# penn-graphics-research/HOT

Hardware: AMD Instinct MI355X
Metric: ms per nonlinear (L-BFGS) iteration; P2G+G2P Mparticles/s; achieved HBM GB/s vs roofline (lower is better)
Workload: dtype f64; 1 GPU; C2: one 63^3-cell cube x 8 ppc (63^3 cells per GPU), fixed-corotated E=50000 nu=0.3, dx=0.01, dt=1/24, -lsolver 3 -mg_level 3 -smoother 5 -coarseSolver 2 --project --linesearch --bcproject --usecn -cneps 1e-7; particles_per_gpu=2000376, particles_total=2000376, nodes_total=267565, levels=3, parallelism=1 GPU

## Files before the change

hot_amd/csrc/mg_build.hip:

```cpp
#include "hot_impl.h"
#include "hot_svd.h"
#include <rocprim/rocprim.hpp>

namespace hot {

__global__ void k_hash_clear2(HashMap h)
{
    uint32_t i = blockIdx.x * blockDim.x + threadIdx.x;
    if (i > h.mask) return;
    h.keys[i] = ~0ULL;
    h.minrank[i] = ~0ULL;
    h.id[i] = -1;
}
__global__ void k_coord_map_insert(HashMap h, const int32_t* __restrict__ coord, int n)
{
    int i = blockIdx.x * blockDim.x + threadIdx.x;
    if (i >= n) return;
    uint32_t s = hash_insert_min(h, coord_key(coord[3 * i], coord[3 * i + 1], coord[3 * i + 2]), (unsigned long long)i);
    h.id[s] = i;
}

__device__ __forceinline__ bool parent_of(const int32_t* __restrict__ coord, int s, int& px, int& py, int& pz)
{
    int i = s >> 3, l = s & 7;
    int x = coord[3 * i], y = coord[3 * i + 1], z = coord[3 * i + 2];
    int dx = l >> 2, dy = (l >> 1) & 1, dz = l & 1;
    if ((dx && !(x & 1)) || (dy && !(y & 1)) || (dz && !(z & 1))) return false;
    px = x / 2 + dx, py = y / 2 + dy, pz = z / 2 + dz;
    return true;
}
__global__ void k_coarse_insert(HashMap h, const int32_t* __restrict__ coord, int n)
{
    int s = blockIdx.x * blockDim.x + threadIdx.x;
    if (s >= n * 8) return;
    int px, py, pz;
    if (parent_of(coord, s, px, py, pz)) hash_insert_min(h, coord_key(px, py, pz), (unsigned long long)s);
}
__global__ void k_coarse_flag(HashMap h, const int32_t* __restrict__ coord, int32_t* flags, int n)
{
    int s = blockIdx.x * blockDim.x + threadIdx.x;
    if (s >= n * 8) return;
    int px, py, pz;
    int f = 0;
    if (parent_of(coord, s, px, py, pz)) {
        int32_t slot = hash_find_slot(h, coord_key(px, py, pz));
        f = h.minrank[slot] == (unsigned long long)s;
    }
    flags[s] = f;
}
__global__ void k_coarse_assign(HashMap h, const int32_t* __restrict__ coord, const int32_t* __restrict__ flags, const int32_t* __restrict__ scan, int32_t* ccoord, int n)
{
    int s = blockIdx.x * blockDim.x + threadIdx.x;
    if (s >= n * 8 || !flags[s]) return;
    int px, py, pz;
    parent_of(coord, s, px, py, pz);
    int id = scan[s];
    h.id[hash_find_slot(h, coord_key(px, py, pz))] = id;
    ccoord[3 * id] = px, ccoord[3 * id + 1] = py, ccoord[3 * id + 2] = pz;
}
template <class T>
__global__ void k_build_P(HashMap cmap, const int32_t* __restrict__ coord, int32_t* pcol, T* pw, int n)
{
    int i = blockIdx.x * blockDim.x + threadIdx.x;
    if (i >= n) return;
    int x = coord[3 * i], y = coord[3 * i + 1], z = coord[3 * i + 2];
    int first = hash_find_id(cmap, coord_key(x / 2, y / 2, z / 2));
    for (int l = 0; l < 8; ++l) {
        int dx = l >> 2, dy = (l >> 1) & 1, dz = l & 1;
        T wx = (x & 1) ? (T)0.5 : (dx ? (T)0 : (T)1), wy = (y & 1) ? (T)0.5 : (dy ? (T)0 : (T)1), wz = (z & 1) ? (T)0.5 : (dz ? (T)0 : (T)1);
        T w = wx * wy * wz;
        int c = first;
        if (w != (T)0) c = hash_find_id(cmap, coord_key(x / 2 + dx, y / 2 + dy, z / 2 + dz));
        pcol[8 * (int64_t)i + l] = c;
        pw[8 * (int64_t)i + l] = w;
    }
}
__global__ void k_build_children(HashMap fmap, const int32_t* __restrict__ ccoord, int32_t* child, int nc)
{
    int e = blockIdx.x * blockDim.x + threadIdx.x;
    if (e >= nc * 27) return;
    int I = e / 27, q = e - I * 27;
    int a = q / 9 - 1, b = (q / 3) % 3 - 1, c = q % 3 - 1;
    int x = 2 * ccoord[3 * I] + a, y = 2 * ccoord[3 * I + 1] + b, z = 2 * ccoord[3 * I + 2] + c;
    child[e] = (x | y | z) < 0 ? -1 : hash_find_id(fmap, coord_key(x, y, z));
}
__global__ void k_coarse_cols(HashMap cmap, const int32_t* __restrict__ ccoord, int32_t* col, int nc)
{
    int64_t e = (int64_t)blockIdx.x * blockDim.x + threadIdx.x;
    if (e >= (int64_t)nc * 125) return;
    int n = (int)(e / 125), k = (int)(e - (int64_t)n * 125);
    int x = ccoord[3 * n] - (k / 25 - 2), y = ccoord[3 * n + 1] - ((k / 5) % 5 - 2), z = ccoord[3 * n + 2] - (k % 5 - 2);
    int j = (x | y | z) < 0 ? -1 : hash_find_id(cmap, coord_key(x, y, z));
    col[e] = j >= 0 ? j : (n > 0 ? 0 : 1);
}

__device__ __forceinline__ void ap_window(int x, int y, int z, int& na, int& nb, int& nc) { na = 3 + (x & 1), nb = 3 + (y & 1), nc = 3 + (z & 1); }
template <class T>
__global__ __launch_bounds__(256) void k_ap(const int32_t* __restrict__ coord, const T* __restrict__ val, T* ap, int n, const uint8_t* __restrict__ own)
{
    __shared__ T row[4][1125];
    int w = threadIdx.x >> 6, lane = threadIdx.x & 63;
    int i = blockIdx.x * 4 + w;
    if (own && i < n && !own[i]) i = n;
    if (i < n) {
        const T* src = val + (int64_t)i * 1125;
        for (int e = lane; e < 1125; e += 64) row[w][e] = src[e];
    }
    __syncthreads();
    if (i >= n) return;
    int x = coord[3 * i], y = coord[3 * i + 1], z = coord[3 * i + 2];
    int cbx = (x - 2) >> 1, cby = (y - 2) >> 1, cbz = (z - 2) >> 1;
    int na, nb, nc;
    ap_window(x, y, z, na, nb, nc);
    const int cnt9 = na * nb * nc * 9;
    for (int o = lane; o < cnt9; o += 64) {
        int js = o / 9, comp = o - js * 9;
        int a = js / (nb * nc), b = (js / nc) % nb, c = js % nc;
        int Jx = cbx + a, Jy = cby + b, Jz = cbz + c;
        T sum = (T)0;
#pragma unroll
        for (int da = -1; da <= 1; ++da) {
            int ddx = x - (2 * Jx + da);
            if (ddx < -2 || ddx > 2) continue;
#pragma unroll
            for (int db = -1; db <= 1; ++db) {
                int ddy = y - (2 * Jy + db);
                if (ddy < -2 || ddy > 2) continue;
#pragma unroll
                for (int dc = -1; dc <= 1; ++dc) {
                    int ddz = z - (2 * Jz + dc);
                    if (ddz < -2 || ddz > 2) continue;
                    T wgt = (da ? (T)0.5 : (T)1) * (db ? (T)0.5 : (T)1) * (dc ? (T)0.5 : (T)1);
                    sum += wgt * row[w][((ddx + 2) * 25 + (ddy + 2) * 5 + (ddz + 2)) * 9 + comp];
                }
            }
        }
        ap[(int64_t)i * 576 + o] = sum;
    }
}
__global__ void k_ap_cols(HashMap cmap, const int32_t* __restrict__ coord, int32_t* apc, int n)
{
    int64_t e = (int64_t)blockIdx.x * blockDim.x + threadIdx.x;
    if (e >= (int64_t)n * 64) return;
    int i = (int)(e >> 6), js = (int)(e & 63);
    int na, nb, nc;
    ap_window(coord[3 * i], coord[3 * i + 1], coord[3 * i + 2], na, nb, nc);
    if ((js >> 4) >= na || ((js >> 2) & 3) >= nb || (js & 3) >= nc) {
        apc[e] = -1;
        return;
    }
    int Jx = ((coord[3 * i] - 2) >> 1) + (js >> 4), Jy = ((coord[3 * i + 1] - 2) >> 1) + ((js >> 2) & 3), Jz = ((coord[3 * i + 2] - 2) >> 1) + (js & 3);
    int j = (Jx | Jy | Jz) < 0 ? -1 : hash_find_id(cmap, coord_key(Jx, Jy, Jz));
    apc[e] = j >= 0 ? j : 0;
}
template <class T>
__global__ __launch_bounds__(256) void k_rap(const int32_t* __restrict__ ccoord, const int32_t* __restrict__ child, const T* __restrict__ ap, T* cval, int nc,
    const uint8_t* __restrict__ fine_own )
{
    __shared__ T sap[9 * 576];
    __shared__ int32_t sci[27];
    const int tid = threadIdx.x, I = blockIdx.x;
    if (tid < 27) {
        const int ci = child[I * 27 + tid];
        sci[tid] = (ci < 0 || (fine_own && !fine_own[ci])) ? -1 : ci;
    }
    int kx[5], ky[5], kz[5], comp[5];
    T sum[5];
#pragma unroll
    for (int t = 0; t < 5; ++t) {
        const int o = min(tid + 256 * t, 1124), k = o / 9;
        comp[t] = o - 9 * k, kx[t] = k / 25, ky[t] = (k / 5) % 5, kz[t] = k % 5, sum[t] = (T)0;
    }
    __syncthreads();
#pragma unroll
    for (int batch = 0; batch < 3; ++batch) {
        for (int e = tid; e < 9 * 576; e += 256) {
            const int q = 9 * batch + e / 576, ci = sci[q];
            const int cnt9 = (3 + (q / 9 != 1)) * (3 + ((q / 3) % 3 != 1)) * (3 + (q % 3 != 1)) * 9;
            if (e % 576 < cnt9) sap[e] = ci >= 0 ? ap[(int64_t)ci * 576 + e % 576] : (T)0;
        }
        __syncthreads();
#pragma unroll
        for (int qq = 0; qq < 9; ++qq) {
            const int q = 9 * batch + qq, da = q / 9 - 1, db = (q / 3) % 3 - 1, dc = q % 3 - 1;
            if (sci[q] < 0) continue;
            const T wgt = (da ? (T)0.5 : (T)1) * (db ? (T)0.5 : (T)1) * (dc ? (T)0.5 : (T)1);
            const int na = 3 + (da != 0), nb = 3 + (db != 0), nc = 3 + (dc != 0);
#pragma unroll
            for (int t = 0; t < 5; ++t) {
                const int a = 3 - kx[t] + (da < 0), bb = 3 - ky[t] + (db < 0), c = 3 - kz[t] + (dc < 0);
                if ((unsigned)a >= (unsigned)na || (unsigned)bb >= (unsigned)nb || (unsigned)c >= (unsigned)nc) continue;
                sum[t] += wgt * sap[qq * 576 + ((a * nb + bb) * nc + c) * 9 + comp[t]];
            }
        }
        __syncthreads();
    }
#pragma unroll
    for (int t = 0; t < 5; ++t)
        if (tid + 256 * t < 1125) cval[(int64_t)I * 1125 + tid + 256 * t] = sum[t];
}

__global__ void k_color_insert(HashMap h, const int32_t* __restrict__ coord, int n)
{
    int i = blockIdx.x * blockDim.x + threadIdx.x;
    if (i >= n) return;
    hash_insert_min(h, coord_key(coord[3 * i] >> 2, coord[3 * i + 1] >> 2, coord[3 * i + 2] >> 2), (unsigned long long)i);
}
__device__ __forceinline__ int color_of(const int32_t* __restrict__ coord, int i)
{
    return (((coord[3 * i] >> 2) & 1) << 2) | (((coord[3 * i + 1] >> 2) & 1) << 1) | ((coord[3 * i + 2] >> 2) & 1);
}
__global__ void k_color_flag(HashMap h, const int32_t* __restrict__ coord, int32_t* flags, int n)
{
    int e = blockIdx.x * blockDim.x + threadIdx.x;
    if (e >= 8 * n) return;
    int c = e / n, i = e - c * n;
    int f = 0;
    if (color_of(coord, i) == c) {
        int32_t slot = hash_find_slot(h, coord_key(coord[3 * i] >> 2, coord[3 * i + 1] >> 2, coord[3 * i + 2] >> 2));
        f = h.minrank[slot] == (unsigned long long)i;
    }
    flags[e] = f;
}
__global__ void k_color_assign(HashMap h, const int32_t* __restrict__ coord, const int32_t* __restrict__ flags, const int32_t* __restrict__ scan, int n)
{
    int e = blockIdx.x * blockDim.x + threadIdx.x;
    if (e >= 8 * n || !flags[e]) return;
    int c = e / n, i = e - c * n;
    int32_t slot = hash_find_slot(h, coord_key(coord[3 * i] >> 2, coord[3 * i + 1] >> 2, coord[3 * i + 2] >> 2));
    h.id[slot] = scan[e] - scan[c * n];
}
__global__ void k_color_keys(HashMap h, const int32_t* __restrict__ coord, uint64_t* keys, uint32_t* vals, int n)
{
    int i = blockIdx.x * blockDim.x + threadIdx.x;
    if (i >= n) return;
    int32_t bid = hash_find_id(h, coord_key(coord[3 * i] >> 2, coord[3 * i + 1] >> 2, coord[3 * i + 2] >> 2));
    keys[i] = ((uint64_t)color_of(coord, i) << 56) | ((uint64_t)(uint32_t)bid << 32) | (uint32_t)i;
    vals[i] = (uint32_t)i;
}
__global__ void k_color_heads(const uint64_t* __restrict__ keys, int32_t* flags, int n)
{
    int p = blockIdx.x * blockDim.x + threadIdx.x;
    if (p >= n) return;
    flags[p] = (p == 0 || (keys[p] >> 32) != (keys[p - 1] >> 32)) ? 1 : 0;
}
__global__ void k_color_finish(const uint64_t* __restrict__ keys, const int32_t* __restrict__ flags, const int32_t* __restrict__ scan, int32_t* gs_order, int32_t* block_start,
    int32_t* color_begin, int n, int nblocks)
{
    int p = blockIdx.x * blockDim.x + threadIdx.x;
    if (p >= n) return;
    gs_order[p] = (int32_t)(keys[p] & 0xffffffffu);
    if (p == 0) block_start[nblocks] = n;
    if (flags[p]) {
        int b = scan[p];
        block_start[b] = p;
        int c = (int)(keys[p] >> 56);
        int cprev = p == 0 ? -1 : (int)(keys[p - 1] >> 56);
        for (int cc = cprev + 1; cc <= c; ++cc) color_begin[cc] = b;
    }
    if (p == n - 1) {
        int c = (int)(keys[p] >> 56);
        for (int cc = c + 1; cc <= 8; ++cc) color_begin[cc] = nblocks;
    }
}
__global__ void k_color_ckey(const uint64_t* __restrict__ keys, const int32_t* __restrict__ scan, const int32_t* __restrict__ block_start, uint32_t* ckey, int n)
{
    int p = blockIdx.x * blockDim.x + threadIdx.x;
    if (p >= n) return;
    int node = (int)(keys[p] & 0xffffffffu);
    int lo = 0, hi = 0;
    (void)lo, (void)hi;
    uint32_t color = (uint32_t)(keys[p] >> 56), bid = (uint32_t)((keys[p] >> 32) & 0xffffff);
    int b = scan[p];
    int start = block_start[b] == p ? p : block_start[b - 1];
    ckey[node] = (color << 28) | (bid << 7) | (uint32_t)(p - start + 1);
}

template <class T>
static void build_coord_map(Ctx<T>* ctx, Level<T>& L)
{
    uint32_t cap = 1024;
    while (cap < 2u * (uint32_t)L.n + 16u) cap <<= 1;
    L.hkeys.reserve(cap), L.hrank.reserve(cap), L.hid.reserve(cap);
    L.map.keys = L.hkeys.p, L.map.minrank = L.hrank.p, L.map.id = L.hid.p, L.map.mask = cap - 1;
    HOT_LAUNCH(ctx, "mg_hash_clear", k_hash_clear2, div_up(cap, 256), 256, 0, L.map);
    HOT_LAUNCH(ctx, "mg_coord_map", k_coord_map_insert, div_up(L.n, 256), 256, 0, L.map, L.coord.p, L.n);
}

struct RankPrefix {
    int v[65];
    uint64_t split[63];
    int R;
};
template <class T>
__global__ void k_color_owner_keys(HashMap h, const int32_t* __restrict__ coord, const int32_t* __restrict__ flags, const int32_t* __restrict__ scan, RankPrefix np, int mode ,
    HashMap block_map, const uint64_t* __restrict__ sharers, const int32_t* __restrict__ child, const uint8_t* __restrict__ fine_owner, uint64_t* __restrict__ keys, uint32_t* __restrict__ vals, int n)
{
    using G = Geo<T>;
    int e = blockIdx.x * blockDim.x + threadIdx.x;
    if (e >= 8 * n || !flags[e]) return;
    const int c = e / n, i = e - c * n;
    const int x = coord[3 * i], y = coord[3 * i + 1], z = coord[3 * i + 2];
    const int32_t slot = hash_find_slot(h, coord_key(x >> 2, y >> 2, z >> 2));
    int r = 0;
    while (r + 1 < np.R && i >= np.v[r + 1]) ++r;
    if (mode == 1) {
        const int hr = home_rank<T>(np.split, np.R, x, y, z, 0);
        int32_t b = hash_find_id(block_map, G::linear_offset(x & ~3, y & ~3, z & ~3) >> 12);
        if (b < 0 && G::BX == 2) b = hash_find_id(block_map, G::linear_offset((x & ~3) + 2, y & ~3, z & ~3) >> 12);
        if (b >= 0 && sharers[b]) {
            const uint64_t sh = sharers[b];
            for (int d = 0; d < np.R; ++d) {
                if (hr - d >= 0 && ((sh >> (hr - d)) & 1ULL)) {
                    r = hr - d;
                    break;
                }
                if (hr + d < np.R && ((sh >> (hr + d)) & 1ULL)) {
                    r = hr + d;
                    break;
                }
            }
        }
    }
    else if (mode == 2) {
        for (int q = 0; q < 27; ++q) {
            const int ci = child[(int64_t)i * 27 + q];
            if (ci >= 0) {
                r = fine_owner[ci];
                break;
            }
        }
    }
    keys[scan[e]] = ((uint64_t)c << 56) | ((uint64_t)r << 48) | (uint32_t)i;
    vals[scan[e]] = (uint32_t)slot;
}
__global__ void k_color_owner_assign(HashMap h, const uint64_t* __restrict__ keys, const uint32_t* __restrict__ slots, const int32_t* __restrict__ scan, uint8_t* __restrict__ owner, int nb, int n)
{
    int p = blockIdx.x * blockDim.x + threadIdx.x;
    if (p >= nb) return;
    const int c = (int)(keys[p] >> 56);
    h.id[slots[p]] = p - scan[(size_t)c * n];
    owner[p] = (uint8_t)((keys[p] >> 48) & 0xff);
}
template <class T>
static void mark_colors(Ctx<T>* ctx, Level<T>& L)
{
    int n = L.n;
    uint32_t cap = 1024;
    while (cap < 2u * (uint32_t)n + 16u) cap <<= 1;
    DBuf<uint64_t>& hk = ctx->col_hk;
    DBuf<unsigned long long>& hr = ctx->col_hr;
    DBuf<int32_t>& hi = ctx->col_hi;
// ... 593 lines not shown
template <class T>
void Ctx<T>::level0_ownership()
{
    release_levels();
    Level<T>* L = acquire_level(0);
    levels.push_back(L);
    L->n = Nn;
    L->coord.reserve(3 * (size_t)Nn);
    HOT_HIP(hipMemcpyAsync(L->coord.p, id2coord.p, 3 * (size_t)Nn * sizeof(int32_t), hipMemcpyDeviceToDevice, stream));
    L->nstart = nstart0;
    {
        IndexPhase ip(this);
        build_coord_map(this, *L);
        color_level(*L);
        level_ownership(*L);
    }
    rebuild_halo(this, 0);
    vmask = L->own.p;
    gs_no_chain = true;
}

typedef double hot_d2 __attribute__((ext_vector_type(2)));
typedef float hot_f4 __attribute__((ext_vector_type(4)));
template <bool NT>
__global__ __launch_bounds__(256) void k_mg32_matrix(const double* __restrict__ in, float* __restrict__ out, size_t n, int* bad)
{
    const size_t i = (size_t)blockIdx.x * 256 + threadIdx.x, n4 = n >> 2;
    bool ok = true;
    if (i < n4) {
        const hot_d2* src = (const hot_d2*)in + 2 * i;
        hot_d2 a, b;
        if constexpr (NT)
            a = __builtin_nontemporal_load(src), b = __builtin_nontemporal_load(src + 1);
        else
            a = src[0], b = src[1];
        hot_f4 f;
        f.x = (float)a.x, f.y = (float)a.y, f.z = (float)b.x, f.w = (float)b.y;
        ok = (f.x - f.x == 0.0f) && (f.y - f.y == 0.0f) && (f.z - f.z == 0.0f) && (f.w - f.w == 0.0f);
        if constexpr (NT)
            __builtin_nontemporal_store(f, (hot_f4*)out + i);
        else
            ((hot_f4*)out)[i] = f;
    }
    else if (i == n4) {
        for (size_t e = 4 * n4; e < n; ++e) {
            const float f = (float)in[e];
            ok = ok && (f - f == 0.0f);
            out[e] = f;
        }
    }
    if (!ok) *bad = 1;
}

template <class T>
void Ctx<T>::check_mixed_allowed()
{
    need(!sharded(), "preconditioner dtype 0 (fp32 hierarchy in an fp64 context) is a single-rank mode: a communicator of size > 1 is not supported with it");
    need(!cfg.useBaselineMultigrid, "preconditioner dtype 0 (fp32 hierarchy in an fp64 context) does not combine with useBaselineMultigrid: its coarse levels are fp64 grids of their own");
    need(!cfg.matrixFree, "preconditioner dtype 0 (fp32 hierarchy in an fp64 context) does not combine with matrixFree: there is no assembled matrix to round");
}
template <class T>
void Ctx<T>::set_preconditioner_dtype(int32_t dtype)
{
    need(dtype == 0 || dtype == 1, "hot_set_preconditioner_dtype: dtype must be 1 (the context's own precision) or 0 (fp32)");
    if (sizeof(T) == 4) {
        need(dtype == 0, "hot_set_preconditioner_dtype: an fp64 hierarchy under an fp32 context is not supported (dtype 1 in a dtype 0 context)");
        return;
    }
    if (dtype == 0) check_mixed_allowed();
    precond_dtype = dtype;
}

template <class T>
void Ctx<T>::build_mg_mixed()
{
    if constexpr (sizeof(T) == 8) {
        need(!levels.empty(), "hot_build_mg before hot_build_hessian");
        check_mixed_allowed();
        need(cfg.systemBCProject != 0, "preconditioner dtype 0 (fp32 hierarchy in an fp64 context) requires systemBCProject: the fp32 smoothers have no boundary projection of their own");
        const double t0 = wall_ms();
        mg32_on = false;
        release_levels(1);
        Level<T>& L0 = *levels[0];
        need(!L0.split, "hot_build_mg with preconditioner dtype 0 after an fp64 hot_build_mg on the same matrix: the fp64 build regrouped the rows of level 0, call hot_build_hessian first");
        if (L0.gs_col.p || L0.residual.p || L0.apv.p) sync(), L0.release_hierarchy();
        for (int id = 0; id < 12; ++id)
            for (size_t k = level_pool[id].size(); k-- > 0;) {
                if (id == 0) {
                    if (level_pool[0][k]->gs_col.p || level_pool[0][k]->apv.p) level_pool[0][k]->release_hierarchy();
                    continue;
                }
                delete level_pool[id][k];
                level_pool[id].erase(level_pool[id].begin() + (long)k);
            }
        if (col_hk.p || cg_dep.p || ap.p)
            sync(), col_hk.release(), col_hr.release(), col_hi.release(), col_cb.release(), cg_dep.release(), ap.release();
        hot_config c32 = cfg;
        c32.dtype = 0;
        if (!mg32) {
            mg32 = new Ctx<float>(c32, stream);
            mg32->in_scale_h = hscal + 252;
            prof_child = mg32;
        }
        mg32->cfg = c32;
        mg32->release_levels(0);
        Level<float>* S = mg32->acquire_level(0);
        mg32->levels.push_back(S);
        const size_t n = (size_t)L0.n, ne = n * 125;
        S->n = L0.n, S->built = false, S->split = false, S->part = false, S->colored = false;
        mg32->Nn = L0.n;
        S->coord.reserve(3 * n), S->col.reserve(ne), S->val.reserve(ne * 9);
        HOT_HIP(hipMemcpyAsync(S->coord.p, L0.coord.p, 3 * n * sizeof(int32_t), hipMemcpyDeviceToDevice, stream));
        HOT_HIP(hipMemcpyAsync(S->col.p, L0.col.p, ne * sizeof(int32_t), hipMemcpyDeviceToDevice, stream));
        int* bad = (int*)(hscal + 253);
        *(volatile int*)bad = 0;
        const int grid = div_up((ne * 9 >> 2) + 1, 256);
        if (ab_flag("HOT_MG32_NT"))
            HOT_LAUNCH(this, "mg32_matrix", k_mg32_matrix<true>, grid, 256, 0, L0.val.p, S->val.p, ne * 9, bad);
        else
            HOT_LAUNCH(this, "mg32_matrix", k_mg32_matrix<false>, grid, 256, 0, L0.val.p, S->val.p, ne * 9, bad);
        mg32->build_diagonal(*S);
        S->nnzb = -1;
        const double before = mg32->stats.ms_mg_build;
        mg32->build_mg();
        mg32->stats.ms_mg_build = before;
        HOT_CHECK(*(volatile int*)bad == 0, HOT_ERR_NUMERIC, "hot_build_mg: an entry of the fp64 matrix is not finite after rounding to fp32 (preconditioner dtype 0)");
        mg32_on = true;
        stats.ms_mg_build += wall_ms() - t0;
    }
}

template <class T>
void Ctx<T>::build_mg()
{
    if (sizeof(T) == 8 && precond_dtype == 0 && !is_shadow) {
        build_mg_mixed();
        return;
    }
    if (mg32_on) drop_mixed();
    need(!levels.empty(), "hot_build_mg before hot_build_hessian");
    need(!(!cfg.systemBCProject && cfg.levelCnt > 1), "levelCnt > 1 requires systemBCProject (ImplicitSolver.h:339)");
    need(cfg.levelCnt >= 1 && cfg.levelCnt <= 10, "levelCnt must be in [1,10] (MultigridPreconditioner.h:369)");
    for (int k : { cfg.smoother, cfg.coarseSolver })
        need(k == 0 || k == 1 || k == 2 || k == 5 || k == 6 || k == 7, "smoother/coarseSolver must be 0, 1, 2, 5, 6 or (coarseSolver only) 7; 3/4 are not selectable in the reference either");
    need(!(cfg.smoother == 7 && cfg.levelCnt > 1), "Do not use IC solver as smoother in the multigrid! (MultigridPreconditioner.h:614,686)");
    need(!(cfg.coarseSolver == 7 && cfg.useBaselineMultigrid), "coarseSolver 7 with useBaselineMultigrid: the baseline fixes its own top solver (MultigridSimulation.inl:447-454)");
    const bool baseline = cfg.useBaselineMultigrid != 0;
    if (baseline) {
        need(!sharded(), "useBaselineMultigrid is a single-rank mode: its coarse levels are whole MPM grids re-rasterised from ALL particles (hot_set_comm with size > 1 is not supported with it)");
        need(cfg.Ainv == 1, "useBaselineMultigrid scales with the inverse diagonal blocks (MultigridSimulation.inl:446): set Ainv = 1");
        need(!cfg.topDownMGS, "useBaselineMultigrid fixes the V-cycle schedule (MultigridSimulation.inl:447-454); topDownMGS does not apply");
    }
    double t0 = wall_ms();
    release_levels(1);
    bool colors = baseline || cfg.smoother == 5 || cfg.coarseSolver == 5 || cfg.coarseSolver == 7 || sharded();
    Level<T>& L0 = *levels[0];
    alloc_work(L0);
    if (colors) color_level(L0);
    if (!baseline && ((cfg.coarseSolver == 6 && cfg.levelCnt == 1) || (cfg.smoother == 6 && cfg.levelCnt > 1))) estimate_2norm(L0, 1e-6);
    for (int level = 0; level < cfg.levelCnt - 1; ++level) {
        Level<T>& F = *levels[level];
        int n = F.n;
        build_coord_map(this, F);
        Level<T>* Cp = acquire_level(level + 1);
        levels.push_back(Cp);
        Level<T>& C = *Cp;
        Ctx<T>* grid = baseline ? build_gmg_grid(level + 1) : nullptr;
        size_t nc;
        if (baseline) {
            Level<T>& G0 = *grid->levels[0];
            C.n = G0.n;
            nc = C.n;
            C.coord.reserve(3 * nc), C.col.reserve(125 * nc), C.val.reserve(1125 * nc), C.child.reserve(27 * nc);
            HOT_HIP(hipMemcpyAsync(C.coord.p, G0.coord.p, 3 * nc * sizeof(int32_t), hipMemcpyDeviceToDevice, stream));
            HOT_HIP(hipMemcpyAsync(C.col.p, G0.col.p, 125 * nc * sizeof(int32_t), hipMemcpyDeviceToDevice, stream));
            HOT_HIP(hipMemcpyAsync(C.val.p, G0.val.p, 1125 * nc * sizeof(T), hipMemcpyDeviceToDevice, stream));
            build_coord_map(this, C);
        }
        else {
            uint32_t cap = 1024;
            while (cap < 2u * (uint32_t)n + 16u) cap <<= 1;
            C.hkeys.reserve(cap), C.hrank.reserve(cap), C.hid.reserve(cap);
            C.map.keys = C.hkeys.p, C.map.minrank = C.hrank.p, C.map.id = C.hid.p, C.map.mask = cap - 1;
            HOT_LAUNCH(this, "mg_hash_clear", k_hash_clear2, div_up(cap, 256), 256, 0, C.map);
            size_t cand = 8 * (size_t)n;
            flags.reserve(cand), scan.reserve(cand);
            HOT_LAUNCH(this, "mg_coarse_insert", k_coarse_insert, div_up(cand, 256), 256, 0, C.map, F.coord.p, n);
            HOT_LAUNCH(this, "mg_coarse_flag", k_coarse_flag, div_up(cand, 256), 256, 0, C.map, F.coord.p, flags.p, n);
            C.n = exclusive_scan_i32(flags.p, scan.p, cand);
            nc = C.n;
            C.coord.reserve(3 * nc), C.col.reserve(125 * nc), C.val.reserve(1125 * nc), C.child.reserve(27 * nc);
            HOT_LAUNCH(this, "mg_coarse_assign", k_coarse_assign, div_up(cand, 256), 256, 0, C.map, F.coord.p, flags.p, scan.p, C.coord.p, n);
            if (sharded()) {
                C.nstart.assign(comm.size + 1, C.n);
                for (int r = 0; r < comm.size; ++r)
                    if (F.nstart[r] < n) HOT_HIP(hipMemcpyAsync(&C.nstart[r], scan.p + 8 * (size_t)F.nstart[r], sizeof(int32_t), hipMemcpyDeviceToHost, stream));
                sync();
            }
        }
        F.pcol.reserve(8 * (size_t)n), F.pw.reserve(8 * (size_t)n);
        HOT_LAUNCH(this, "mg_build_P", k_build_P<T>, div_up(n, 256), 256, 0, C.map, F.coord.p, F.pcol.p, F.pw.p, n);
        HOT_LAUNCH(this, "mg_build_children", k_build_children, div_up(27 * nc, 256), 256, 0, F.map, C.coord.p, C.child.p, C.n);
        if (baseline) {
            HOT_HIP(hipMemsetAsync(dscal.p + 210, 0, sizeof(double), stream));
            HOT_LAUNCH(this, "gmg_check_parents", k_count_missing_parents, div_up(8 * (size_t)n, 256), 256, 0, F.pcol.p, 8 * (int64_t)n, (int32_t*)(dscal.p + 210));
            int32_t missing = 0;
            HOT_HIP(hipMemcpyAsync(&missing, dscal.p + 210, sizeof(int32_t), hipMemcpyDeviceToHost, stream));
            sync();
            need(missing == 0, "useBaselineMultigrid: a fine node has a trilinear parent that is not a DOF of the coarse grid");
        }
        else
            HOT_LAUNCH(this, "mg_coarse_cols", k_coarse_cols, div_up(125 * nc, 256), 256, 0, C.map, C.coord.p, C.col.p, C.n);
        F.apv.reserve(576 * (size_t)n), F.apc.reserve(64 * (size_t)n);
        HOT_LAUNCH(this, "mg_AP", k_ap<T>, div_up(n, 4), 256, 0, F.coord.p, F.val.p, F.apv.p, n, F.mask());
        HOT_LAUNCH(this, "mg_AP_cols", k_ap_cols, div_up(64 * (size_t)n, 256), 256, 0, C.map, F.coord.p, F.apc.p, n);
        if (!baseline) HOT_LAUNCH(this, "mg_RAP", k_rap<T>, nc, 256, 0, C.coord.p, C.child.p, F.apv.p, C.val.p, C.n, F.mask());
        if (F.part) {
            const int minrows = comm.partition_min_rows > 0 ? comm.partition_min_rows : 4096;
            if (C.n >= minrows) {
                color_level(C);
                level_ownership(C);
                DBuf<uint8_t> touched;
                touched.reserve(nc);
                HOT_LAUNCH(this, "shard_coarse_touched", k_coarse_touched, div_up(nc, 256), 256, 0, C.child.p, F.own.p, touched.p, C.n);
                exchange_rows(C, touched.p);
                if (halo_mode()) rebuild_halo(this, level + 1), rebuild_halo(this, level);
            }
            else {
                CommTag tag(this, "coarse_matrix_allreduce");
                c_allreduce(C.val.p, (int64_t)nc * 1125, REAL, HOT_COMM_SUM, true);
            }
        }
        build_diagonal(C);
        C.nnzb = -1;
        alloc_work(C);
        if (colors) color_level(C);
        if (!baseline && ((cfg.coarseSolver == 6 && level + 2 == cfg.levelCnt) || (cfg.smoother == 6 && level + 2 < cfg.levelCnt))) estimate_2norm(C, 1e-6);
        if (colors) split_rows(this, F);
    }
    if (cfg.coarseSolver == 7) {
        Level<T>& Top = *levels.back();
        build_ic(Top);
        Top.ic_rowcnt.reserve(4 * (size_t)Top.n), Top.ic_pad.reserve(512 * (size_t)Top.nblocks);
        HOT_LAUNCH(this, "gs_split_rows", k_gs_split_rows<T>, div_up(Top.n, 4), 256, 0, Top.ic_col.p, Top.ic_val.p, Top.ckey.p, Top.ic_rowcnt.p, Top.n, (const uint8_t*)nullptr, (int32_t*)nullptr, (int32_t*)nullptr);
        HOT_LAUNCH(this, "gs_pad", k_gs_pad, div_up((size_t)Top.nblocks * 64, 256), 256, 0, Top.gs_block_start.p, Top.gs_order.p, Top.ic_rowcnt.p, Top.ic_pad.p, Top.nblocks, (const int32_t*)nullptr);
    }
    if (colors) split_rows(this, *levels.back());
    sync();
    stats.ms_mg_build += wall_ms() - t0;
}

template <class T>
void Ctx<T>::get_level(int32_t level, int32_t* nrows, int32_t* colsize, int32_t* ic)
{
    if (mixed() && level >= 1) {
        mg32->get_level(level, nrows, colsize, ic);
        return;
    }
    need(level >= 0 && level < (int)levels.size(), "level out of range");
    Level<T>& L = *levels[level];
    if (nrows) *nrows = L.n;
    if (colsize) *colsize = 125;
    download(ic, L.coord.p, 3 * (size_t)L.n);
    sync();
}
template <class T>
void Ctx<T>::get_matrix(int32_t level, int32_t* entryCol, void* entryVal)
{
    if constexpr (sizeof(T) == 8)
        if (mixed() && level >= 1) {
            need(level < nlevels(), "level out of range");
            Level<float>& S = *mg32->levels[level];
            DBuf<T> w;
            w.reserve(1125 * (size_t)S.n);
            widen_dev(1125 * (size_t)S.n, S.val.p, w.p);
            download(entryCol, S.col.p, 125 * (size_t)S.n);
            download(entryVal, w.p, 1125 * (size_t)S.n);
            sync();
            return;
        }
    need(level >= 0 && level < (int)levels.size(), "level out of range");
    Level<T>& L = *levels[level];
    download(entryCol, L.col.p, 125 * (size_t)L.n);
    download(entryVal, L.val.p, 1125 * (size_t)L.n);
    sync();
}
template <class T>
void Ctx<T>::get_prolongation(int32_t level, int32_t* entryCol, void* weight)
{
    if constexpr (sizeof(T) == 8)
        if (mixed()) {
            need(level >= 0 && level + 1 < nlevels(), "level out of range");
            Level<float>& S = *mg32->levels[level];
            DBuf<T> w;
            w.reserve(8 * (size_t)S.n);
            widen_dev(8 * (size_t)S.n, S.pw.p, w.p);
            download(entryCol, S.pcol.p, 8 * (size_t)S.n);
            download(weight, w.p, 8 * (size_t)S.n);
            sync();
            return;
        }
    need(level >= 0 && level + 1 < (int)levels.size(), "level out of range");
    Level<T>& L = *levels[level];
    download(entryCol, L.pcol.p, 8 * (size_t)L.n);
    download(weight, L.pw.p, 8 * (size_t)L.n);
    sync();
}

template struct Ctx<float>;
template struct Ctx<double>;

}
```

Baseline: 2.958 ms/iter.

## Restructure Galerkin AP and RAP kernels with constexpr stencil tables and vector loads

Rewrites the multigrid setup kernels k_ap and k_rap. k_ap now reads compile-time tables of contributing stencil runs per parity class and skips structurally-zero terms. It uses 16-byte vector loads into shared memory and a wave barrier in place of a block barrier. k_rap loads child AP rows as vectors into registers, double-buffers them into shared memory across batches, and uses precomputed masks so each thread covers a yz slot across all 5 kx. These kernels only run while the hierarchy is built, so their effect on per-iteration time depends on how often the Hessian and multigrid are rebuilt.

```diff
diff --git a/hot_amd/csrc/ab_src/mg_build_ab1.hip b/hot_amd/csrc/ab_src/mg_build_ab1.hip
--- /dev/null
+++ b/hot_amd/csrc/ab_src/mg_build_ab1.hip
@@ -0,0 +1,89 @@
+template <class T>
+__global__ __launch_bounds__(256) void k_ap_v1(const int32_t* __restrict__ coord, const T* __restrict__ val, T* ap, int n, const uint8_t* __restrict__ own)
+{
+    __shared__ T row[4][1125];
+    int w = threadIdx.x >> 6, lane = threadIdx.x & 63;
+    int i = blockIdx.x * 4 + w;
+    if (own && i < n && !own[i]) i = n;
+    if (i < n) {
+        const T* src = val + (int64_t)i * 1125;
+        for (int e = lane; e < 1125; e += 64) row[w][e] = src[e];
+    }
+    __syncthreads();
+    if (i >= n) return;
+    int x = coord[3 * i], y = coord[3 * i + 1], z = coord[3 * i + 2];
+    int cbx = (x - 2) >> 1, cby = (y - 2) >> 1, cbz = (z - 2) >> 1;
+    int na, nb, nc;
+    ap_window(x, y, z, na, nb, nc);
+    const int cnt9 = na * nb * nc * 9;
+    for (int o = lane; o < cnt9; o += 64) {
+        int js = o / 9, comp = o - js * 9;
+        int a = js / (nb * nc), b = (js / nc) % nb, c = js % nc;
+        int Jx = cbx + a, Jy = cby + b, Jz = cbz + c;
+        T sum = (T)0;
+#pragma unroll
+        for (int da = -1; da <= 1; ++da) {
+            int ddx = x - (2 * Jx + da);
+            if (ddx < -2 || ddx > 2) continue;
+#pragma unroll
+            for (int db = -1; db <= 1; ++db) {
+                int ddy = y - (2 * Jy + db);
+                if (ddy < -2 || ddy > 2) continue;
+#pragma unroll
+                for (int dc = -1; dc <= 1; ++dc) {
+                    int ddz = z - (2 * Jz + dc);
+                    if (ddz < -2 || ddz > 2) continue;
+                    T wgt = (da ? (T)0.5 : (T)1) * (db ? (T)0.5 : (T)1) * (dc ? (T)0.5 : (T)1);
+                    sum += wgt * row[w][((ddx + 2) * 25 + (ddy + 2) * 5 + (ddz + 2)) * 9 + comp];
+                }
+            }
+        }
+        ap[(int64_t)i * 576 + o] = sum;
+    }
+}
+template <class T>
+__global__ __launch_bounds__(256) void k_rap_v1(const int32_t* __restrict__ ccoord, const int32_t* __restrict__ child, const T* __restrict__ ap, T* cval, int nc,
+    const uint8_t* __restrict__ fine_own )
+{
+    __shared__ T sap[9 * 576];
+    __shared__ int32_t sci[27];
+    const int tid = threadIdx.x, I = blockIdx.x;
+    if (tid < 27) {
+        const int ci = child[I * 27 + tid];
+        sci[tid] = (ci < 0 || (fine_own && !fine_own[ci])) ? -1 : ci;
+    }
+    int kx[5], ky[5], kz[5], comp[5];
+    T sum[5];
+#pragma unroll
+    for (int t = 0; t < 5; ++t) {
+        const int o = min(tid + 256 * t, 1124), k = o / 9;
+        comp[t] = o - 9 * k, kx[t] = k / 25, ky[t] = (k / 5) % 5, kz[t] = k % 5, sum[t] = (T)0;
+    }
+    __syncthreads();
+#pragma unroll
+    for (int batch = 0; batch < 3; ++batch) {
+        for (int e = tid; e < 9 * 576; e += 256) {
+            const int q = 9 * batch + e / 576, ci = sci[q];
+            const int cnt9 = (3 + (q / 9 != 1)) * (3 + ((q / 3) % 3 != 1)) * (3 + (q % 3 != 1)) * 9;
+            if (e % 576 < cnt9) sap[e] = ci >= 0 ? ap[(int64_t)ci * 576 + e % 576] : (T)0;
+        }
+        __syncthreads();
+#pragma unroll
+        for (int qq = 0; qq < 9; ++qq) {
+            const int q = 9 * batch + qq, da = q / 9 - 1, db = (q / 3) % 3 - 1, dc = q % 3 - 1;
+            if (sci[q] < 0) continue;
+            const T wgt = (da ? (T)0.5 : (T)1) * (db ? (T)0.5 : (T)1) * (dc ? (T)0.5 : (T)1);
+            const int na = 3 + (da != 0), nb = 3 + (db != 0), nc = 3 + (dc != 0);
+#pragma unroll
+            for (int t = 0; t < 5; ++t) {
+                const int a = 3 - kx[t] + (da < 0), bb = 3 - ky[t] + (db < 0), c = 3 - kz[t] + (dc < 0);
+                if ((unsigned)a >= (unsigned)na || (unsigned)bb >= (unsigned)nb || (unsigned)c >= (unsigned)nc) continue;
+                sum[t] += wgt * sap[qq * 576 + ((a * nb + bb) * nc + c) * 9 + comp[t]];
+            }
+        }
+        __syncthreads();
+    }
+#pragma unroll
+    for (int t = 0; t < 5; ++t)
+        if (tid + 256 * t < 1125) cval[(int64_t)I * 1125 + tid + 256 * t] = sum[t];
+}
diff --git a/hot_amd/csrc/mg_build.hip b/hot_amd/csrc/mg_build.hip
--- a/hot_amd/csrc/mg_build.hip
+++ b/hot_amd/csrc/mg_build.hip
@@ -1,5 +1,6 @@
 #include "hot_impl.h"
 #include "hot_svd.h"
+#include "mg_galerkin_tables.h"
 #include <rocprim/rocprim.hpp>
 
 namespace hot {
@@ -95,47 +96,69 @@
 }
 
 __device__ __forceinline__ void ap_window(int x, int y, int z, int& na, int& nb, int& nc) { na = 3 + (x & 1), nb = 3 + (y & 1), nc = 3 + (z & 1); }
+#ifdef HOT_AB_KERNELS
+#include "ab_src/mg_build_ab1.hip"
+#endif
+__device__ constexpr galerkin::ApTables ap_tables = galerkin::make_ap_tables();
 template <class T>
 __global__ __launch_bounds__(256) void k_ap(const int32_t* __restrict__ coord, const T* __restrict__ val, T* ap, int n, const uint8_t* __restrict__ own)
 {
-    __shared__ T row[4][1125];
-    int w = threadIdx.x >> 6, lane = threadIdx.x & 63;
-    int i = blockIdx.x * 4 + w;
-    if (own && i < n && !own[i]) i = n;
-    if (i < n) {
-        const T* src = val + (int64_t)i * 1125;
-        for (int e = lane; e < 1125; e += 64) row[w][e] = src[e];
-    }
-    __syncthreads();
-    if (i >= n) return;
-    int x = coord[3 * i], y = coord[3 * i + 1], z = coord[3 * i + 2];
-    int cbx = (x - 2) >> 1, cby = (y - 2) >> 1, cbz = (z - 2) >> 1;
-    int na, nb, nc;
-    ap_window(x, y, z, na, nb, nc);
-    const int cnt9 = na * nb * nc * 9;
+    using galerkin::ApPos;
+    constexpr int V = 16 / (int)sizeof(T);
+    typedef T piece __attribute__((ext_vector_type(V)));
+    constexpr int ROW = (1125 + 2 * (V - 1)) / V * V;
+    constexpr int NLOAD = (ROW / V + 63) / 64;
+    __shared__ __attribute__((aligned(16))) T row[4][ROW];
+    __shared__ uint32_t order[4][64];
+    const int w = __builtin_amdgcn_readfirstlane(threadIdx.x >> 6), lane = threadIdx.x & 63;
+    const int i = blockIdx.x * 4 + w;
+    if (i >= n || (own && !own[i])) return;
+    const T* src = val + (int64_t)i * 1125;
+    const int shift = (int)(((uintptr_t)src & 15) / sizeof(T)), head = shift ? V - shift : 0;
+    const int npiece = (1125 - head) / V, tail = head + npiece * V;
+    T* r = row[w] + shift;
+    const int x = coord[3 * i], y = coord[3 * i + 1], z = coord[3 * i + 2];
+    const int cls = __builtin_amdgcn_readfirstlane(((x & 1) << 2) | ((y & 1) << 1) | (z & 1));
+    const int cnt9 = ((3 + (x & 1)) * (3 + (y & 1)) * (3 + (z & 1))) * 9;
+    {
+        piece p[NLOAD];
+        const uint32_t e = ap_tables.pos[cls][lane];
+#pragma unroll
+        for (int k = 0; k < NLOAD; ++k)
+            if (lane + 64 * k < npiece) p[k] = *(const piece*)(src + head + (lane + 64 * k) * V);
+        if (lane < head) r[lane] = src[lane];
+        if (tail + lane < 1125) r[tail + lane] = src[tail + lane];
+#pragma unroll
+        for (int k = 0; k < NLOAD; ++k)
+            if (lane + 64 * k < npiece) *(piece*)(r + head + (lane + 64 * k) * V) = p[k];
+        order[w][lane] = e;
+    }
+    T* dst = ap + (int64_t)i * 576;
+    __builtin_amdgcn_fence(__ATOMIC_RELEASE, "wavefront");
+    __builtin_amdgcn_wave_barrier();
+    __builtin_amdgcn_fence(__ATOMIC_ACQUIRE, "wavefront");
+    int pos = lane / 9, comp = lane - 9 * pos;
     for (int o = lane; o < cnt9; o += 64) {
-        int js = o / 9, comp = o - js * 9;
-        int a = js / (nb * nc), b = (js / nc) % nb, c = js % nc;
-        int Jx = cbx + a, Jy = cby + b, Jz = cbz + c;
+        const uint32_t e = order[w][pos];
+        const T* q = r + ApPos::base(e) + comp;
+        const int nx = ApPos::count(e, 0), ny = ApPos::count(e, 1), nz = ApPos::count(e, 2);
+        const int fx = ApPos::first(e, 0), fy = ApPos::first(e, 1), fz = ApPos::first(e, 2);
+        const T w0 = fz ? (T)0.5 : (T)1, w1 = fz + 1 ? (T)0.5 : (T)1, w2 = fz + 2 ? (T)0.5 : (T)1;
         T sum = (T)0;
-#pragma unroll
-        for (int da = -1; da <= 1; ++da) {
-            int ddx = x - (2 * Jx + da);
-            if (ddx < -2 || ddx > 2) continue;
-#pragma unroll
-            for (int db = -1; db <= 1; ++db) {
-                int ddy = y - (2 * Jy + db);
-                if (ddy < -2 || ddy > 2) continue;
-#pragma unroll
-                for (int dc = -1; dc <= 1; ++dc) {
-                    int ddz = z - (2 * Jz + dc);
-                    if (ddz < -2 || ddz > 2) continue;
-                    T wgt = (da ? (T)0.5 : (T)1) * (db ? (T)0.5 : (T)1) * (dc ? (T)0.5 : (T)1);
-                    sum += wgt * row[w][((ddx + 2) * 25 + (ddy + 2) * 5 + (ddz + 2)) * 9 + comp];
-                }
-            }
-        }
-        ap[(int64_t)i * 576 + o] = sum;
+        for (int a = 0; a < nx; ++a) {
+            const T wa = fx + a ? (T)0.5 : (T)1;
+            for (int b = 0; b < ny; ++b) {
+                const T wab = wa * (fy + b ? (T)0.5 : (T)1);
+                const T* p = q - (225 * a + 45 * b);
+                const T v0 = p[0], v1 = nz > 1 ? p[-9] : (T)0, v2 = nz > 2 ? p[-18] : (T)0;
+                sum = fma(wab * w0, v0, sum);
+                sum = fma(wab * w1, v1, sum);
+                sum = fma(wab * w2, v2, sum);
+            }
+        }
+        dst[ApPos::slot(e) * 9 + comp] = sum;
+        pos += 7, comp += 1;
+        if (comp == 9) comp = 0, pos += 1;
     }
 }
 __global__ void k_ap_cols(HashMap cmap, const int32_t* __restrict__ coord, int32_t* apc, int n)
@@ -157,47 +180,74 @@
 __global__ __launch_bounds__(256) void k_rap(const int32_t* __restrict__ ccoord, const int32_t* __restrict__ child, const T* __restrict__ ap, T* cval, int nc,
     const uint8_t* __restrict__ fine_own )
 {
-    __shared__ T sap[9 * 576];
+    namespace g = galerkin;
+    constexpr int V = 16 / (int)sizeof(T);
+    typedef T piece __attribute__((ext_vector_type(V)));
+    constexpr int NSLOT = (576 / V + 255) / 256;
+    __shared__ __attribute__((aligned(16))) T sap[9 * 576];
     __shared__ int32_t sci[27];
+    __shared__ uint32_t shave;
     const int tid = threadIdx.x, I = blockIdx.x;
-    if (tid < 27) {
-        const int ci = child[I * 27 + tid];
-        sci[tid] = (ci < 0 || (fine_own && !fine_own[ci])) ? -1 : ci;
-    }
-    int kx[5], ky[5], kz[5], comp[5];
-    T sum[5];
-#pragma unroll
-    for (int t = 0; t < 5; ++t) {
-        const int o = min(tid + 256 * t, 1124), k = o / 9;
-        comp[t] = o - 9 * k, kx[t] = k / 25, ky[t] = (k / 5) % 5, kz[t] = k % 5, sum[t] = (T)0;
-    }
+    if (tid < 64) {
+        int ci = -1;
+        if (tid < 27) {
+            ci = child[I * 27 + tid];
+            if (ci >= 0 && fine_own && !fine_own[ci]) ci = -1;
+            sci[tid] = ci;
+        }
+        const unsigned long long have = __ballot(ci >= 0);
+        if (tid == 0) shave = (uint32_t)have;
+    }
+    const int o2 = tid < 225 ? tid : 0, k2 = o2 / 9, comp = o2 - 9 * k2, ky = k2 / 5, kz = k2 - 5 * ky;
+    const uint32_t terms = tid < 225 ? g::rap_mask_yz(ky, kz) : 0u;
+    const int at[2] = { comp - 9 * (ky * 3 + kz), comp - 9 * (ky * 4 + kz) };
+    T sum[5] = { (T)0, (T)0, (T)0, (T)0, (T)0 };
     __syncthreads();
+    const uint32_t have = __builtin_amdgcn_readfirstlane(shave);
+    piece held[9][NSLOT];
+    auto load = [&](int batch) {
+#pragma unroll
+        for (int qq = 0; qq < 9; ++qq) {
+            const int q = 9 * batch + qq, npiece = (g::rap_child_scalars(q) + V - 1) / V;
+            if (!(have >> q & 1u)) continue;
+            const piece* src = (const piece*)(ap + (int64_t)__builtin_amdgcn_readfirstlane(sci[q]) * 576);
+#pragma unroll
+            for (int s = 0; s < NSLOT; ++s)
+                if (256 * (s + 1) <= npiece || tid + 256 * s < npiece) held[qq][s] = src[tid + 256 * s];
+        }
+        asm volatile("" ::: "memory");
+    };
+    auto store = [&](int batch) {
+#pragma unroll
+        for (int qq = 0; qq < 9; ++qq) {
+            const int q = 9 * batch + qq, npiece = (g::rap_child_scalars(q) + V - 1) / V;
+            if (!(have >> q & 1u)) continue;
+#pragma unroll
+            for (int s = 0; s < NSLOT; ++s)
+                if (256 * (s + 1) <= npiece || tid + 256 * s < npiece) ((piece*)(sap + qq * 576))[tid + 256 * s] = held[qq][s];
+        }
+    };
+    load(0);
 #pragma unroll
     for (int batch = 0; batch < 3; ++batch) {
-        for (int e = tid; e < 9 * 576; e += 256) {
-            const int q = 9 * batch + e / 576, ci = sci[q];
-            const int cnt9 = (3 + (q / 9 != 1)) * (3 + ((q / 3) % 3 != 1)) * (3 + (q % 3 != 1)) * 9;
-            if (e % 576 < cnt9) sap[e] = ci >= 0 ? ap[(int64_t)ci * 576 + e % 576] : (T)0;
-        }
+        store(batch);
         __syncthreads();
+        if (batch < 2) load(batch + 1);
 #pragma unroll
         for (int qq = 0; qq < 9; ++qq) {
             const int q = 9 * batch + qq, da = q / 9 - 1, db = (q / 3) % 3 - 1, dc = q % 3 - 1;
-            if (sci[q] < 0) continue;
             const T wgt = (da ? (T)0.5 : (T)1) * (db ? (T)0.5 : (T)1) * (dc ? (T)0.5 : (T)1);
-            const int na = 3 + (da != 0), nb = 3 + (db != 0), nc = 3 + (dc != 0);
-#pragma unroll
-            for (int t = 0; t < 5; ++t) {
-                const int a = 3 - kx[t] + (da < 0), bb = 3 - ky[t] + (db < 0), c = 3 - kz[t] + (dc < 0);
-                if ((unsigned)a >= (unsigned)na || (unsigned)bb >= (unsigned)nb || (unsigned)c >= (unsigned)nc) continue;
-                sum[t] += wgt * sap[qq * 576 + ((a * nb + bb) * nc + c) * 9 + comp[t]];
-            }
-        }
-        __syncthreads();
-    }
-#pragma unroll
-    for (int t = 0; t < 5; ++t)
-        if (tid + 256 * t < 1125) cval[(int64_t)I * 1125 + tid + 256 * t] = sum[t];
+            if (!(have >> q & 1u) || !(terms >> qq & 1u)) continue;
+            const T* row = sap + qq * 576 + g::rap_child_const(q) + at[g::rap_child_n(q, 2) - 3];
+#pragma unroll
+            for (int kx = 0; kx < 5; ++kx)
+                if (g::rap_valid(kx, da)) sum[kx] = fma(wgt, row[-9 * kx * g::rap_child_n(q, 1) * g::rap_child_n(q, 2)], sum[kx]);
+        }
+        if (batch < 2) __syncthreads();
+    }
+    if (tid < 225)
+#pragma unroll
+        for (int kx = 0; kx < 5; ++kx) cval[(int64_t)I * 1125 + 225 * kx + tid] = sum[kx];
 }
 
 __global__ void k_color_insert(HashMap h, const int32_t* __restrict__ coord, int n)
@@ -1097,6 +1147,7 @@
         need(!cfg.topDownMGS, "useBaselineMultigrid fixes the V-cycle schedule (MultigridSimulation.inl:447-454); topDownMGS does not apply");
     }
     double t0 = wall_ms();
+    [[maybe_unused]] const bool galerkin_v1 = ab_flag("HOT_GALERKIN_V1");
     release_levels(1);
     bool colors = baseline || cfg.smoother == 5 || cfg.coarseSolver == 5 || cfg.coarseSolver == 7 || sharded();
     Level<T>& L0 = *levels[0];
@@ -1157,9 +1208,19 @@
         else
             HOT_LAUNCH(this, "mg_coarse_cols", k_coarse_cols, div_up(125 * nc, 256), 256, 0, C.map, C.coord.p, C.col.p, C.n);
         F.apv.reserve(576 * (size_t)n), F.apc.reserve(64 * (size_t)n);
-        HOT_LAUNCH(this, "mg_AP", k_ap<T>, div_up(n, 4), 256, 0, F.coord.p, F.val.p, F.apv.p, n, F.mask());
+#ifdef HOT_AB_KERNELS
+        if (galerkin_v1)
+            HOT_LAUNCH(this, lname("mg_AP_v1", level).c_str(), k_ap_v1<T>, div_up(n, 4), 256, 0, F.coord.p, F.val.p, F.apv.p, n, F.mask());
+        else
+#endif
+            HOT_LAUNCH(this, lname("mg_AP", level).c_str(), k_ap<T>, div_up(n, 4), 256, 0, F.coord.p, F.val.p, F.apv.p, n, F.mask());
         HOT_LAUNCH(this, "mg_AP_cols", k_ap_cols, div_up(64 * (size_t)n, 256), 256, 0, C.map, F.coord.p, F.apc.p, n);
-        if (!baseline) HOT_LAUNCH(this, "mg_RAP", k_rap<T>, nc, 256, 0, C.coord.p, C.child.p, F.apv.p, C.val.p, C.n, F.mask());
+#ifdef HOT_AB_KERNELS
+        if (!baseline && galerkin_v1)
+            HOT_LAUNCH(this, lname("mg_RAP_v1", level).c_str(), k_rap_v1<T>, nc, 256, 0, C.coord.p, C.child.p, F.apv.p, C.val.p, C.n, F.mask());
+        else
+#endif
+            if (!baseline) HOT_LAUNCH(this, lname("mg_RAP", level).c_str(), k_rap<T>, nc, 256, 0, C.coord.p, C.child.p, F.apv.p, C.val.p, C.n, F.mask());
         if (F.part) {
             const int minrows = comm.partition_min_rows > 0 ? comm.partition_min_rows : 4096;
             if (C.n >= minrows) {
diff --git a/hot_amd/csrc/mg_galerkin_tables.h b/hot_amd/csrc/mg_galerkin_tables.h
--- /dev/null
+++ b/hot_amd/csrc/mg_galerkin_tables.h
@@ -0,0 +1,128 @@
+#pragma once
+#include <cstdint>
+
+namespace hot {
+namespace galerkin {
+
+constexpr int ap_positions(int par) { return 3 + par; }
+constexpr int ap_dist(int par, int a, int d) { return par + 2 - 2 * a - d; }
+constexpr bool ap_valid(int par, int a, int d) { return ap_dist(par, a, d) >= -2 && ap_dist(par, a, d) <= 2; }
+constexpr int ap_count(int par, int a) { return (int)ap_valid(par, a, -1) + (int)ap_valid(par, a, 0) + (int)ap_valid(par, a, 1); }
+constexpr int ap_first(int par, int a) { return ap_valid(par, a, -1) ? -1 : ap_valid(par, a, 0) ? 0 : 1; }
+constexpr int ap_stencil(int par, int a, int d) { return ap_dist(par, a, d) + 2; }
+constexpr bool ap_is_run(int par, int a)
+{
+    for (int d = -1; d <= 1; ++d)
+        if (ap_valid(par, a, d) != (d >= ap_first(par, a) && d < ap_first(par, a) + ap_count(par, a))) return false;
+    return true;
+}
+constexpr int ap_axis_terms(int par)
+{
+    int s = 0;
+    for (int a = 0; a < ap_positions(par); ++a) s += ap_count(par, a);
+    return s;
+}
+static_assert(ap_count(0, 0) == 2 && ap_count(0, 1) == 3 && ap_count(0, 2) == 2 && ap_count(0, 3) == 0, "even coordinate: (2, 3, 2) terms, position 3 structurally zero");
+static_assert(ap_count(1, 0) == 1 && ap_count(1, 1) == 3 && ap_count(1, 2) == 3 && ap_count(1, 3) == 1, "odd coordinate: (1, 3, 3, 1) terms");
+static_assert(ap_is_run(0, 0) && ap_is_run(0, 1) && ap_is_run(0, 2) && ap_is_run(1, 0) && ap_is_run(1, 1) && ap_is_run(1, 2) && ap_is_run(1, 3), "valid d are contiguous");
+static_assert(ap_axis_terms(0) == 7 && ap_axis_terms(1) == 8, "");
+static_assert(ap_axis_terms(0) * ap_axis_terms(0) * ap_axis_terms(0) == 343 && ap_axis_terms(1) * ap_axis_terms(1) * ap_axis_terms(1) == 512, "343 .. 512 terms per row and component");
+
+struct ApPos {
+    static constexpr uint32_t pack(int px, int py, int pz, int a, int b, int c)
+    {
+        const int slot = (a * ap_positions(py) + b) * ap_positions(pz) + c;
+        const int fx = ap_first(px, a), fy = ap_first(py, b), fz = ap_first(pz, c);
+        const int base = (ap_stencil(px, a, fx) * 25 + ap_stencil(py, b, fy) * 5 + ap_stencil(pz, c, fz)) * 9;
+        return (uint32_t)slot | (uint32_t)base << 6 | (uint32_t)ap_count(px, a) << 17 | (uint32_t)ap_count(py, b) << 19 | (uint32_t)ap_count(pz, c) << 21 | (uint32_t)(fx + 1) << 23
+            | (uint32_t)(fy + 1) << 25 | (uint32_t)(fz + 1) << 27;
+    }
+    static constexpr int slot(uint32_t e) { return (int)(e & 63u); }
+    static constexpr int base(uint32_t e) { return (int)(e >> 6 & 2047u); }
+    static constexpr int count(uint32_t e, int axis) { return (int)(e >> (17 + 2 * axis) & 3u); }
+    static constexpr int first(uint32_t e, int axis) { return (int)(e >> (23 + 2 * axis) & 3u) - 1; }
+    static constexpr int terms(uint32_t e) { return count(e, 0) * count(e, 1) * count(e, 2); }
+};
+struct ApTables {
+    uint32_t pos[8][64];
+    int32_t npos[8];
+    int32_t steps[8];
+};
+constexpr ApTables make_ap_tables()
+{
+    ApTables t{};
+    for (int cls = 0; cls < 8; ++cls) {
+        const int px = cls >> 2, py = (cls >> 1) & 1, pz = cls & 1;
+        int n = 0;
+        for (int a = 0; a < ap_positions(px); ++a)
+            for (int b = 0; b < ap_positions(py); ++b)
+                for (int c = 0; c < ap_positions(pz); ++c) {
+                    const uint32_t e = ApPos::pack(px, py, pz, a, b, c);
+                    int at = n++;
+                    for (; at > 0 && ApPos::terms(t.pos[cls][at - 1]) < ApPos::terms(e); --at) t.pos[cls][at] = t.pos[cls][at - 1];
+                    t.pos[cls][at] = e;
+                }
+        t.npos[cls] = n;
+        for (int o = 0; o < 9 * n; o += 64) t.steps[cls] += ApPos::terms(t.pos[cls][o / 9]);
+    }
+    return t;
+}
+constexpr int ap_class_terms(const ApTables& t, int cls)
+{
+    int s = 0;
+    for (int p = 0; p < t.npos[cls]; ++p) s += ApPos::terms(t.pos[cls][p]);
+    return s;
+}
+constexpr bool ap_tables_ok(const ApTables& t)
+{
+    for (int cls = 0; cls < 8; ++cls) {
+        const int odd = (cls >> 2) + ((cls >> 1) & 1) + (cls & 1);
+        int want = 1, npos = 1;
+        for (int k = 0; k < 3; ++k) want *= k < odd ? 8 : 7, npos *= k < odd ? 4 : 3;
+        if (ap_class_terms(t, cls) != want || t.npos[cls] != npos) return false;
+        for (int p = 1; p < t.npos[cls]; ++p)
+            if (ApPos::terms(t.pos[cls][p - 1]) < ApPos::terms(t.pos[cls][p])) return false;
+        if (64 * t.steps[cls] >= 2 * 9 * want) return false;
+    }
+    return true;
+}
+static_assert(ap_tables_ok(make_ap_tables()), "per class: 7^e 8^o terms, 3^e 4^o positions, longest first");
+
+constexpr int rap_position(int k, int d) { return 3 - k + (d < 0 ? 1 : 0); }
+constexpr bool rap_valid(int k, int d) { return rap_position(k, d) >= 0 && rap_position(k, d) < 3 + (d != 0 ? 1 : 0); }
+constexpr uint32_t rap_axis_mask(int k) { return (rap_valid(k, -1) ? 1u : 0u) | (rap_valid(k, 0) ? 2u : 0u) | (rap_valid(k, 1) ? 4u : 0u); }
+constexpr int popc3(uint32_t m) { return (int)((m & 1u) + (m >> 1 & 1u) + (m >> 2 & 1u)); }
+static_assert(popc3(rap_axis_mask(0)) == 1 && popc3(rap_axis_mask(1)) == 3 && popc3(rap_axis_mask(2)) == 3 && popc3(rap_axis_mask(3)) == 3 && popc3(rap_axis_mask(4)) == 1,
+    "slot k has 1, 3, 3, 3, 1 contributing children per axis");
+static_assert(rap_axis_mask(0) == 4u && rap_axis_mask(4) == 1u, "the outermost slots: only the child on their own side");
+constexpr uint32_t RAP_AXIS = rap_axis_mask(0) | rap_axis_mask(1) << 3 | rap_axis_mask(2) << 6 | rap_axis_mask(3) << 9 | rap_axis_mask(4) << 12;
+constexpr uint32_t rap_mask_yz(int ky, int kz)
+{
+    const uint32_t my = RAP_AXIS >> (3 * ky) & 7u, mz = RAP_AXIS >> (3 * kz) & 7u;
+    return ((my & 1u) ? mz : 0u) | ((my & 2u) ? mz << 3 : 0u) | ((my & 4u) ? mz << 6 : 0u);
+}
+constexpr uint32_t rap_mask(int kx, int ky, int kz)
+{
+    uint32_t m = 0;
+    for (int da = -1; da <= 1; ++da)
+        if (rap_valid(kx, da)) m |= rap_mask_yz(ky, kz) << (9 * (da + 1));
+    return m;
+}
+constexpr int rap_total_terms()
+{
+    int s = 0;
+    for (int k = 0; k < 125; ++k)
+        for (int q = 0; q < 27; ++q) s += (int)(rap_mask(k / 25, (k / 5) % 5, k % 5) >> q & 1u);
+    return s;
+}
+static_assert(rap_total_terms() == 11 * 11 * 11, "10.6 of 27 children per slot on average");
+constexpr int rap_child_n(int q, int axis) { return 3 + ((axis == 0 ? q / 9 : axis == 1 ? (q / 3) % 3 : q % 3) != 1 ? 1 : 0); }
+constexpr int rap_child_scalars(int q) { return rap_child_n(q, 0) * rap_child_n(q, 1) * rap_child_n(q, 2) * 9; }
+constexpr int rap_child_const(int q)
+{
+    const int da = q / 9 - 1, db = (q / 3) % 3 - 1, dc = q % 3 - 1, nb = rap_child_n(q, 1), nc = rap_child_n(q, 2);
+    return 9 * ((rap_position(0, da) * nb + rap_position(0, db)) * nc + rap_position(0, dc));
+}
+
+}
+}
```

Result: no change. 2.964 ms/iter (median of 2 runs) (+0.2%).
